# MaxMax2016/MixGAN-TTS

Hardware: AMD Instinct MI355X
Metric: denoiser steps/sec (80-mel, L=1000 frames, B=16 per GPU) (higher is better)
Workload: dtype f32

## Files before the change

### mixgan-tts_amd/csrc/denoiser_persist.h

```cpp
#pragma once
#include "common.h"
#include "denoiser_common.h"
#include "resblock_fused.h"

#define DP_SPIN_LIMIT (1u << 21)
#define DP_F_ROLES 1
#define DP_F_WITHHOLD 2

typedef unsigned long long dp_u64;
typedef __attribute__((address_space(1))) dp_u64 dp_gu64;
typedef __attribute__((address_space(1))) unsigned dp_gu32;
typedef __attribute__((address_space(1))) const char dp_gcchar;
typedef __attribute__((address_space(1))) const f32x4 dp_gcf32x4;

struct PersistArgs {
    const float *x_t;
    const float *cond;
    const float *cproj;
    float *cproj_out;
    const float *in_w, *in_b;
    const float *layers;
    size_t layer_stride, l_wc, l_w3, l_wo, l_bc, l_b3, l_bo;
    const float *p16layers;
    size_t p16layer_stride, p_wc, p_w3, p_wo;
    const float *skip_w, *skip_b, *out_w, *out_b;
    const float *hvec, *dvec;
    int vec_rows;
    float *out;
    const int64_t *t;
    const float *coef1, *coef2, *logvar;
    const float *noise;
    unsigned long long seed;
    unsigned long long noise_stream;
    float *x0_out;
    dp_u64 *gran;
    dp_u64 *team;
    unsigned *sync;
    unsigned *host_err;
    unsigned spin_limit;
    float *x0_save, *y_save, *skip_save;
    float *h_save, *g_save, *sig_save, *tnh_save;
    size_t act_stride;
    unsigned long long *dbg;
    int dbg_wave;
    int B, L, M, NL, tiles_per_b, post, clip, n_steps;
    int flags;
    float rsNL;
    int b_split;
    const float *x_t2, *hvec2, *dvec2, *cond2;
    float *out2;
};

struct DpIterK1 {
    static constexpr int N = 8, KW = 1;
    static __device__ __forceinline__ int chunk(int it) { return it; }
    static __device__ __forceinline__ int tap(int) { return 0; }
};
struct DpIterHead {
    static constexpr int N = 3, KW = 1;
    static __device__ __forceinline__ int chunk(int it) { return it; }
    static __device__ __forceinline__ int tap(int) { return 0; }
};
struct DpIterCentre {
    static constexpr int N = 8, KW = 3;
    static __device__ __forceinline__ int chunk(int it) { return it; }
    static __device__ __forceinline__ int tap(int) { return 1; }
};
struct DpIterOuter {
    static constexpr int N = 16, KW = 3;
    static __device__ __forceinline__ int chunk(int it) { return it >> 1; }
    static __device__ __forceinline__ int tap(int it) { return (it & 1) * 2; }
};

__device__ __forceinline__ int dp_pos(int ch) { return ((ch & 1) << 2) | ((ch >> 1) & 3); }
template <int NTC>
__device__ __forceinline__ int dp_at(int ch, int col) { return (((ch >> 3) * NTC + col) << 3) + dp_pos(ch); }

#ifndef DP_DIST_BIG
#define DP_DIST_BIG 3
#endif
template <int NMB, int NNB, int NTC, class IT, int DIST, bool SBASE>
__device__ __forceinline__ void dp_mfma_loop_at(f32x16 (&acc)[NMB][NNB], const f32x4 *const (&ap)[NMB], unsigned loff,
                                                const float *__restrict__ tile)
{
    static_assert(DIST >= 1 && DIST <= 3, "ring of 4 slots");
    f32x4 ring[4][NMB];
    f32x4 bb[2][NNB];
    dp_gcchar *ub[NMB];
    if (SBASE) {
#pragma unroll
        for (int i = 0; i < NMB; ++i) {
            const unsigned long long v = reinterpret_cast<unsigned long long>(ap[i]);
            const unsigned lo = __builtin_amdgcn_readfirstlane((unsigned)v), hi = __builtin_amdgcn_readfirstlane((unsigned)(v >> 32));
            ub[i] = (dp_gcchar *)(((unsigned long long)hi << 32) | lo);
        }
    }
    auto sbase = [&](int i, int qb) {
        dp_gcchar *p = ub[i] + (size_t)qb * 1024;
        asm volatile("" : "+s"(p));
        return p;
    };
    if (SBASE) asm volatile("" : "+v"(loff));
    auto wload = [&](int i, int qb, int d) -> f32x4 {
        if (SBASE) return *(dp_gcf32x4 *)(ub[i] + (size_t)qb * 1024 + loff + d * 1024);
        return ap[i][(size_t)(qb + d) * 64];
    };
    auto qbase = [](int it) { return (IT::chunk(it) * IT::KW + IT::tap(it)) * 4; };
    auto boff = [](int it) { return IT::chunk(it) * (4 * NTC * 8) + IT::tap(it) * 8; };
    {
        const int q0 = qbase(0);
#pragma unroll
        for (int s = 0; s < DIST; ++s)
#pragma unroll
            for (int i = 0; i < NMB; ++i) ring[s][i] = wload(i, q0, s);
        const float *T0 = tile + boff(0);
#pragma unroll
        for (int j = 0; j < NNB; ++j) bb[0][j] = *reinterpret_cast<const f32x4 *>(T0 + 32 * 8 * j);
    }
#pragma unroll 1
    for (int it = 0; it < IT::N; ++it) {
        const int itn = it + 1 < IT::N ? it + 1 : IT::N - 1;
        const int qc = qbase(it), qn = qbase(itn);
        const float *Tc = tile + boff(it), *Tn = tile + boff(itn);
        dp_gcchar *bc[NMB], *bn[NMB];
        if (SBASE) {
            asm volatile("" : "+v"(loff));
#pragma unroll
            for (int i = 0; i < NMB; ++i) {
                bc[i] = sbase(i, qc);
                bn[i] = sbase(i, qn);
            }
        }
#pragma unroll
        for (int u = 0; u < 4; ++u) {
#pragma unroll
            for (int i = 0; i < NMB; ++i) {
                constexpr int LIM = 4 - DIST;
                const int d = u < LIM ? u + DIST : u - LIM;
                if (SBASE) ring[(u + DIST) & 3][i] = *(dp_gcf32x4 *)((u < LIM ? bc[i] : bn[i]) + loff + d * 1024);
                else ring[(u + DIST) & 3][i] = wload(i, u < LIM ? qc : qn, d);
            }
            {
                const float *Tx = u < 3 ? Tc + (u + 1) * (NTC * 8) : Tn;
#pragma unroll
                for (int j = 0; j < NNB; ++j) bb[(u + 1) & 1][j] = *reinterpret_cast<const f32x4 *>(Tx + 32 * 8 * j);
            }
            __builtin_amdgcn_sched_barrier(0);
#pragma unroll
            for (int e = 0; e < 4; ++e) {
#pragma unroll
                for (int i = 0; i < NMB; ++i)
#pragma unroll
                    for (int j = 0; j < NNB; ++j)
                        acc[i][j] = __builtin_amdgcn_mfma_f32_32x32x2f32(ring[u][i][e], bb[u & 1][j][e], acc[i][j], 0, 0, 0);
                if (NMB * NNB < 4) __builtin_amdgcn_sched_barrier(0);
            }
            __builtin_amdgcn_sched_barrier(0);
        }
    }
}
template <int NMB, int NNB, int NTC, class IT, int DIST = (NMB * NNB >= 4 ? DP_DIST_BIG : 3)>
__device__ __forceinline__ void dp_mfma_loop(f32x16 (&acc)[NMB][NNB], const f32x4 *const (&ap)[NMB], const float *__restrict__ tile)
{
    dp_mfma_loop_at<NMB, NNB, NTC, IT, DIST, false>(acc, ap, 0u, tile);
}
template <int NMB, int NNB, int NTC, class IT, int DIST = (NMB * NNB >= 4 ? DP_DIST_BIG : 3)>
__device__ __forceinline__ void dp_mfma_loop_sbase(f32x16 (&acc)[NMB][NNB], const f32x4 *const (&ap)[NMB], unsigned loff,
                                             const float *__restrict__ tile)
{
    dp_mfma_loop_at<NMB, NNB, NTC, IT, DIST, true>(acc, ap, loff, tile);
}

template <int NTC, class F>
__device__ __forceinline__ void dp_store_block(float *T, int ch0, int col, int hh, F val)
{
#pragma unroll
    for (int q = 0; q < 4; ++q) {
        float *base = T + ((((ch0 >> 3) + q) * NTC + col) << 3);
        const f32x2 lo = {val(4 * q + 0), val(4 * q + 2)}, hi = {val(4 * q + 1), val(4 * q + 3)};
        *reinterpret_cast<f32x2 *>(base + 2 * hh) = lo;
        *reinterpret_cast<f32x2 *>(base + 4 + 2 * hh) = hi;
    }
}

__device__ __forceinline__ void dp_philox(unsigned long long seed, unsigned long long offset, unsigned long long idx,
                                          unsigned (&r)[4])
{
    unsigned c0 = (unsigned)idx, c1 = (unsigned)(idx >> 32), c2 = (unsigned)offset, c3 = (unsigned)(offset >> 32);
    unsigned k0 = (unsigned)seed, k1 = (unsigned)(seed >> 32);
#pragma unroll
    for (int i = 0; i < 10; ++i) {
        const unsigned long long p0 = (unsigned long long)0xD2511F53u * c0, p1 = (unsigned long long)0xCD9E8D57u * c2;
        const unsigned n0 = (unsigned)(p1 >> 32) ^ c1 ^ k0, n1 = (unsigned)p1, n2 = (unsigned)(p0 >> 32) ^ c3 ^ k1,
                       n3 = (unsigned)p0;
        c0 = n0; c1 = n1; c2 = n2; c3 = n3;
        k0 += 0x9E3779B9u;
        k1 += 0xBB67AE85u;
    }
    r[0] = c0; r[1] = c1; r[2] = c2; r[3] = c3;
}

__device__ __forceinline__ float dp_normal(unsigned long long seed, unsigned long long offset, unsigned long long idx)
{
    unsigned r[4];
    dp_philox(seed, offset, idx, r);
    const float u1 = ((float)r[0] + 1.0f) * 2.3283064365386963e-10f;
    const float u2 = (float)r[1] * 2.3283064365386963e-10f;
    return sqrtf(-2.0f * __logf(u1)) * __cosf(6.283185307179586f * u2);
}

#define DP_RLX_AGENT __ATOMIC_RELAXED, __HIP_MEMORY_SCOPE_AGENT

__device__ __forceinline__ void dp_fail(unsigned *sync, unsigned *host_err, unsigned code)
{
    __hip_atomic_store(sync + DP_SYNC_ERROR, code, DP_RLX_AGENT);
    if (host_err) __hip_atomic_store(host_err, code, __ATOMIC_RELAXED, __HIP_MEMORY_SCOPE_SYSTEM);
    __builtin_amdgcn_fence(__ATOMIC_RELEASE, "agent");
}
__device__ __forceinline__ bool dp_failed(unsigned *sync)
{
    __builtin_amdgcn_fence(__ATOMIC_ACQUIRE, "agent");
    return __hip_atomic_load(sync + DP_SYNC_ERROR, DP_RLX_AGENT) != 0u;
}
__device__ __forceinline__ void dp_take_ticket(int tid, unsigned *sync, unsigned &s_ticket, unsigned &s_launch, unsigned &s_dead)
{
    if (tid == 0) {
        s_ticket = __hip_atomic_fetch_add(sync + DP_SYNC_TICKET, 1u, DP_RLX_AGENT);
        s_launch = __hip_atomic_load(sync + DP_SYNC_LAUNCHES, DP_RLX_AGENT);
        s_dead = 0u;
    }
}
template <bool QUEUE_B>
__device__ __forceinline__ void dp_retire(int tid, unsigned *sync, int n_slots)
{
    if (tid == 0) {
        const unsigned done = __hip_atomic_fetch_add(sync + DP_SYNC_DONE, 1u, DP_RLX_AGENT);
        if (done == (unsigned)n_slots - 1u) {
            __hip_atomic_store(sync + DP_SYNC_DONE, 0u, DP_RLX_AGENT);
            __hip_atomic_store(sync + DP_SYNC_TICKET, 0u, DP_RLX_AGENT);
            if (QUEUE_B) __hip_atomic_store(sync + DP_SYNC_TICKET_B, 0u, DP_RLX_AGENT);
            __hip_atomic_fetch_add(sync + DP_SYNC_LAUNCHES, 1u, DP_RLX_AGENT);
        }
    }
}
#define DP_EPOCH(launch_no, NL, step) ((launch_no) * ((unsigned)(NL) + 1u) + (unsigned)(step) + 1u)

struct DpPosterior { float c1, c2, sg; };
__device__ __forceinline__ DpPosterior dp_posterior_at(const PersistArgs &a, int b)
{
    long tb = (long)a.t[b];
    tb = tb < 0 ? 0 : (tb >= a.n_steps ? a.n_steps - 1 : tb);
    const float c1 = a.coef1[tb], c2 = a.coef2[tb];
    const float sg = tb == 0 ? 0.f : __expf(0.5f * a.logvar[tb]);
    return {c1, c2, sg};
}
__device__ __forceinline__ float dp_clip_x0(float x0, int clip)
{
    if (clip) x0 = fminf(fmaxf(x0, -1.f), 1.f);
    return x0;
}
__device__ __forceinline__ float dp_posterior(const DpPosterior &p, float x0, float xt, float nz) { return fmaf(p.sg, nz, fmaf(p.c1, x0, p.c2 * xt)); }
#define DP_STAMP(k) do { if (TIMING && tid == 64 * a.dbg_wave) a.dbg[((size_t)tile * (a.NL + 2) + stamp_row) * 12 + (k)] = clock64(); } while (0)

template <int NT, int RW>
__device__ __forceinline__ void dp_cproj_fetch(const float *cp, float *cl, int w, int lane, int l0, int L)
{
    constexpr int LPR = NT / 4;
    constexpr int RPI = 64 / LPR;
    const int rsub = lane / LPR, c4 = lane - rsub * LPR;
    unsigned off = (unsigned)(((RW * w + rsub) * L + min(l0 + 4 * c4, L - 4)) * 4);
    asm volatile("" : "+v"(off));
    float *dst = cl + (size_t)RW * w * NT;
    const unsigned at = (unsigned)(size_t)(__attribute__((address_space(3))) void *)dst;
#pragma unroll
    for (int it = 0; it < RW / RPI; ++it) {
        const float *gi = cp + (size_t)it * RPI * L;
        const unsigned m = __builtin_amdgcn_readfirstlane(at + (unsigned)(it * RPI * NT * 4));
        asm volatile("s_mov_b32 m0, %0\n\ts_nop 0\n\tglobal_load_lds_dwordx4 %1, %2" : : "s"(m), "v"(off), "s"(gi) : "memory");
    }
}

template <int NT, bool VEC4, bool TIMING = false, bool SAVE = false, int NWV = NT / 8, int CPM = 0, bool SOLO = false>
__global__ __launch_bounds__(NWV * 64, ((NT == 64 && NWV == 4) || SOLO) ? 1 : 2) void denoiser_persist_kernel(PersistArgs a)
{
    static_assert(!SOLO || (NT == 32 && NWV == 4), "SOLO is the one-per-CU build of the 4-wave 32-frame form");
    static_assert(!(CPM && SAVE), "the saving forward computes its projections and keeps none");
    constexpr bool READP = CPM == 2, WRITEP = CPM == 1;
#ifndef DP_DIST_SOLO
#define DP_DIST_SOLO 2
#endif
    constexpr int DBIG = ((NT == 64 && NWV == 4) || SOLO) ? DP_DIST_SOLO : DP_DIST_BIG;
#ifndef DP_ONEPASS_WHEN
#define DP_ONEPASS_WHEN (MB == 2 && ((NT == 64 && NWV == 4) || SOLO))
#endif
    static_assert((NT == 32 && (NWV == 4 || NWV == 8)) || (NT == 64 && (NWV == 8 || NWV == 4)),
                  "tile widths: 32 frames (4 waves, two workgroups per CU; or 8 waves, one per CU) or 64 (8 waves, one)");
    constexpr int NTHR = NWV * 64, NW = NWV;
    constexpr bool TWO_PER_CU = NT == 32 && NWV == 4;
    constexpr int MB = 8 / NW;
    constexpr bool ONEPASS = DP_ONEPASS_WHEN;
    constexpr int NNB = NT / 32;
    constexpr int NC = NT, NH = NT + 2;
    __shared__ __attribute__((aligned(16))) float lds[RB_C * (NC + NH)];
    __shared__ unsigned s_tile, s_dead, s_launch;
    float *condT = lds;
    float *hT = lds + RB_C * NC;

    const int tid = threadIdx.x, lane = tid & 63, w = tid >> 6;
    const int hh = lane >> 5, c32 = lane & 31;
    const int L = a.L;
    const int wu = __builtin_amdgcn_readfirstlane(w);
    const unsigned loff = (unsigned)lane * 16u;

    const int n_tiles = a.tiles_per_b * a.B;
    const unsigned hw_id = __builtin_amdgcn_s_getreg((31 << 11) | 4);
    const int role = (TWO_PER_CU && (a.flags & DP_F_ROLES)) ? (int)(hw_id & 1u) : 0;
    if (tid == 0) {
        const int nA = (TWO_PER_CU && (a.flags & DP_F_ROLES)) ? (a.B / 2) * a.tiles_per_b : n_tiles;
        const int n_mine = role == 0 ? nA : n_tiles - nA;
        unsigned tk = __hip_atomic_fetch_add(a.sync + (role ? DP_SYNC_TICKET_B : DP_SYNC_TICKET), 1u, DP_RLX_AGENT);
        int tl;
        if ((int)tk < n_mine) tl = (role == 0 ? 0 : nA) + (int)tk;
        else {
            tk = __hip_atomic_fetch_add(a.sync + (role ? DP_SYNC_TICKET : DP_SYNC_TICKET_B), 1u, DP_RLX_AGENT);
            tl = (role == 0 ? nA : 0) + (int)tk;
        }
        s_tile = (unsigned)tl;
        s_launch = __hip_atomic_load(a.sync + DP_SYNC_LAUNCHES, DP_RLX_AGENT);
        s_dead = 0u;
    }
    __syncthreads();
    const int tile = min((int)s_tile, n_tiles - 1);
    const unsigned launch_no = s_launch;
    const int bg = tile / a.tiles_per_b, jt = tile - bg * a.tiles_per_b;
    const bool second = a.b_split > 0 && bg >= a.b_split;
    const int b = second ? bg - a.b_split : bg;
    const int Bp = a.b_split > 0 ? (second ? a.B - a.b_split : a.b_split) : a.B;
    const bool do_save = SAVE && (a.b_split == 0 || second);
    const float *const x_in = second ? a.x_t2 : a.x_t;
    float *const x_out = second ? a.out2 : a.out;
    const int l0 = jt * NT;
    const bool has_left = jt > 0, has_right = jt + 1 < a.tiles_per_b;
    int stamp_row = 0;
    DP_STAMP(0);
    if (TIMING && tid == 0) {
        a.dbg[((size_t)tile * (a.NL + 2)) * 12 + 2] = hw_id;
        a.dbg[((size_t)tile * (a.NL + 2)) * 12 + 3] = __builtin_amdgcn_s_getreg((31 << 11) | 20);
    }

    {
        const float *cb = (second ? a.cond2 : a.cond) + (size_t)b * RB_C * L;
        if (READP) {
            if (VEC4) dp_cproj_fetch<NT, 32 * MB>(a.cproj + (size_t)b * a.NL * RB_C * L, lds, w, lane, l0, L);
        } else if (VEC4) {
#pragma unroll
            for (int k = 0; k < 64 * NT / NTHR; ++k) {
                const int idx = tid + k * NTHR;
                const int row = idx / (NT / 4), c4 = idx - row * (NT / 4);
                const int f0 = l0 + 4 * c4;
                const bool ok = f0 < L;
                const f32x4 v = *reinterpret_cast<const f32x4 *>(cb + (size_t)row * L + min(f0, L - 4));
#pragma unroll
                for (int e = 0; e < 4; ++e) condT[dp_at<NC>(row, 4 * c4 + e)] = ok ? v[e] : 0.f;
            }
        } else {
#pragma unroll
            for (int k = 0; k < 256 * NT / NTHR; ++k) {
                const int idx = tid + k * NTHR;
                const int row = idx / NT, cc = idx - row * NT;
                const int f = l0 + cc;
                const float v = cb[(size_t)row * L + min(f, L - 1)];
                condT[dp_at<NC>(row, cc)] = f < L ? v : 0.f;
            }
        }
        const float *xb = x_in + (size_t)b * a.M * L;
#pragma unroll
        for (int k = 0; k < 96 * NT / NTHR; ++k) {
            const int idx = tid + k * NTHR;
            const int row = idx / NT, c = idx - row * NT;
            const int f = l0 + c;
            const float v = xb[(size_t)min(row, a.M - 1) * L + min(f, L - 1)];
            hT[dp_at<NH>(row, c)] = (row < a.M && f < L) ? v : 0.f;
        }
    }

    f32x16 st[2 * MB][NNB];
    const int rbase = 32 * MB * w;
    auto row_of = [&](int i, int r) { return rbase + 32 * i + 8 * (r >> 2) + 4 * hh + (r & 3); };
#pragma unroll
    for (int i = 0; i < MB; ++i)
#pragma unroll
        for (int j = 0; j < NNB; ++j)
#pragma unroll
            for (int r = 0; r < 16; ++r) {
                st[i][j][r] = a.in_b[row_of(i, r)];
                st[MB + i][j][r] = 0.f;
            }
    __syncthreads();
    {
        f32x16 acc[MB][NNB];
        const f32x4 *ap[MB];
#pragma unroll
        for (int i = 0; i < MB; ++i) {
            ap[i] = reinterpret_cast<const f32x4 *>(a.in_w) + (size_t)(MB * wu + i) * 12 * 64;
#pragma unroll
            for (int j = 0; j < NNB; ++j) acc[i][j] = st[i][j];
        }
        dp_mfma_loop_sbase<MB, NNB, NH, DpIterHead>(acc, ap, loff, hT + c32 * 8 + hh * 4);
#pragma unroll
        for (int i = 0; i < MB; ++i)
#pragma unroll
            for (int j = 0; j < NNB; ++j)
#pragma unroll
                for (int r = 0; r < 16; ++r) st[i][j][r] = fmaxf(acc[i][j][r], 0.f);
    }
    DP_STAMP(1);
    bool fvalid[NNB];
    const size_t bbase = (size_t)b * RB_C * L;
    auto save_block = [&](float *dst, int ch0, int j, auto val) {
        const int f = l0 + 32 * j + c32;
        if (f < L) {
#pragma unroll
            for (int r = 0; r < 16; ++r) dst[bbase + (size_t)(ch0 + 8 * (r >> 2) + 4 * hh + (r & 3)) * L + f] = val(r);
        }
    };
#pragma unroll
    for (int j = 0; j < NNB; ++j) fvalid[j] = l0 + 32 * j + c32 < L;
    if (SAVE && do_save) {
#pragma unroll
        for (int i = 0; i < MB; ++i)
#pragma unroll
            for (int j = 0; j < NNB; ++j) save_block(a.x0_save, rbase + 32 * i, j, [&](int r) { return st[i][j][r]; });
    }
    dp_gu64 *const gran = (dp_gu64 *)a.gran;

    for (int l = 0; l < a.NL; ++l) {
        const float *lp = a.layers + (size_t)l * a.layer_stride;
        const size_t vrows = a.vec_rows ? (size_t)a.vec_rows : (size_t)Bp;
        const float *hv = (second ? a.hvec2 : a.hvec) + ((size_t)l * vrows + b) * RB_C;
        const float *dv = (second ? a.dvec2 : a.dvec) + ((size_t)l * vrows + b) * RB_C;
        const unsigned epoch = DP_EPOCH(launch_no, a.NL, l);
        const int par = l & 1;
        stamp_row = l + 1;
        DP_STAMP(0);

        f32x16 acc1[MB][NNB];
        if (READP && VEC4) {
            asm volatile("s_waitcnt vmcnt(0)" ::: "memory");
#pragma unroll
            for (int i = 0; i < MB; ++i)
#pragma unroll
                for (int j = 0; j < NNB; ++j)
#pragma unroll
                    for (int r = 0; r < 16; ++r) acc1[i][j][r] = lds[row_of(i, r) * NT + 32 * j + c32];
        } else if (READP) {
            const float *cp = a.cproj + ((size_t)b * a.NL + l) * RB_C * L;
#pragma unroll
            for (int i = 0; i < MB; ++i)
#pragma unroll
                for (int j = 0; j < NNB; ++j) {
                    unsigned lo = (unsigned)((rbase + 4 * hh) * L + min(l0 + 32 * j + c32, L - 1));
                    asm volatile("" : "+v"(lo));
#pragma unroll
                    for (int r = 0; r < 16; ++r) acc1[i][j][r] = cp[lo + (unsigned)((32 * i + 8 * (r >> 2) + (r & 3)) * L)];
                }
        } else {
#pragma unroll
            for (int i = 0; i < MB; ++i)
#pragma unroll
                for (int j = 0; j < NNB; ++j)
#pragma unroll
                    for (int r = 0; r < 16; ++r) acc1[i][j][r] = lp[a.l_bc + row_of(i, r)];
            const f32x4 *wc = reinterpret_cast<const f32x4 *>(lp + a.l_wc);
            const f32x4 *ap[MB];
#pragma unroll
            for (int i = 0; i < MB; ++i) ap[i] = wc + (size_t)(MB * wu + i) * 32 * 64;
            dp_mfma_loop_sbase<MB, NNB, NC, DpIterK1, (MB * NNB >= 4 ? DBIG : 3)>(acc1, ap, loff, condT + c32 * 8 + hh * 4);
            if (WRITEP) {
                float *co = a.cproj_out + ((size_t)b * a.NL + l) * RB_C * L;
                unsigned lo = (unsigned)((rbase + 4 * hh) * L + l0 + c32);
                asm volatile("" : "+v"(lo));
#pragma unroll
                for (int i = 0; i < MB; ++i)
#pragma unroll
                    for (int j = 0; j < NNB; ++j)
                        if (l0 + 32 * j + c32 < L) {
#pragma unroll
                            for (int r = 0; r < 16; ++r)
                                co[lo + (unsigned)((32 * i + 8 * (r >> 2) + (r & 3)) * L + 32 * j)] = acc1[i][j][r];
                        }
            }
        }
#pragma unroll
        for (int i = 0; i < MB; ++i)
#pragma unroll
            for (int j = 0; j < NNB; ++j)
#pragma unroll
                for (int r = 0; r < 16; ++r) acc1[i][j][r] += st[i][j][r] + hv[row_of(i, r)];
        DP_STAMP(1);
        f32x16 acc2[MB][2][NNB];
#pragma unroll
        for (int p = 0; p < MB; ++p)
#pragma unroll
            for (int r = 0; r < 16; ++r) {
                const int ch = row_of(p, r);
                const float bg = lp[a.l_b3 + ch], bf = lp[a.l_b3 + RB_C + ch];
#pragma unroll
                for (int j = 0; j < NNB; ++j) {
                    acc2[p][0][j][r] = bg;
                    acc2[p][1][j][r] = bf;
                }
            }
        __syncthreads();
        DP_STAMP(2);
#pragma unroll
        for (int i = 0; i < MB; ++i)
#pragma unroll
            for (int j = 0; j < NNB; ++j)
            {
                dp_store_block<NH>(hT, rbase + 32 * i, 1 + 32 * j + c32, hh,
                                   [&](int r) { return fvalid[j] ? acc1[i][j][r] : 0.f; });
                if (SAVE && do_save) save_block(a.h_save + (size_t)l * a.act_stride, rbase + 32 * i, j, [&](int r) { return acc1[i][j][r]; });
            }
        if (READP && VEC4 && l + 1 < a.NL)
            dp_cproj_fetch<NT, 32 * MB>(a.cproj + ((size_t)b * a.NL + l + 1) * RB_C * L, lds, w, lane, l0, L);
        __syncthreads();
        DP_STAMP(3);

        if (w < 2) {
            bool go = w == 0 ? has_left : has_right;
            if ((a.flags & DP_F_WITHHOLD) && w == 0 && jt == 1) go = false;
            if (go) {
                const int dst_tile = w == 0 ? tile - 1 : tile + 1;
                const int col = w == 0 ? 1 : NT;
                dp_gu64 *g = gran + (((size_t)par * n_tiles + dst_tile) * 2 + (w == 0 ? 1 : 0)) * RB_C;
#pragma unroll
                for (int k = 0; k < 4; ++k) {
                    const int row = lane + 64 * k;
                    const dp_u64 v = ((dp_u64)epoch << 32) | (dp_u64)__float_as_uint(hT[dp_at<NH>(row, col)]);
                    __hip_atomic_store(g + row, v, DP_RLX_AGENT);
                }
            }
        }

        const f32x4 *w3 = reinterpret_cast<const f32x4 *>(lp + a.l_w3);
        const f32x4 *ap2[MB][2];
#pragma unroll
        for (int p = 0; p < MB; ++p) {
            ap2[p][0] = w3 + (size_t)(2 * (MB * wu + p)) * 96 * 64;
            ap2[p][1] = w3 + (size_t)(2 * (MB * wu + p) + 1) * 96 * 64;
        }
        if (ONEPASS) {
            dp_mfma_loop_sbase<2 * MB, NNB, NH, DpIterCentre, DBIG>(reinterpret_cast<f32x16 (&)[2 * MB][NNB]>(acc2),
                                                              reinterpret_cast<const f32x4 *const (&)[2 * MB]>(ap2), loff,
                                                              hT + c32 * 8 + hh * 4);
        } else {
#pragma unroll
            for (int p = 0; p < MB; ++p)
                dp_mfma_loop_sbase<2, NNB, NH, DpIterCentre, (2 * NNB >= 4 ? DBIG : 3)>(acc2[p], ap2[p], loff, hT + c32 * 8 + hh * 4);
        }
        DP_STAMP(4);

        if (w < 2) {
            const bool from = w == 0 ? has_left : has_right;
            const int col = w == 0 ? 0 : NT + 1;
            unsigned v[4] = {0u, 0u, 0u, 0u};
            if (from && s_dead == 0u) {
                dp_gu64 *g = gran + (((size_t)par * n_tiles + tile) * 2 + w) * RB_C;
                unsigned spins = 0;
                for (;;) {
                    bool ok = true;
#pragma unroll
                    for (int k = 0; k < 4; ++k) {
                        const dp_u64 x = __hip_atomic_load(g + lane + 64 * k, DP_RLX_AGENT);
                        v[k] = (unsigned)x;
                        ok &= (unsigned)(x >> 32) == epoch;
                    }
                    if (__all(ok)) break;
                    if (++spins > a.spin_limit) {
                        if (lane == 0) {
                            dp_fail(a.sync, a.host_err, 1u + (unsigned)l);
                            s_dead = 1u;
                        }
                        break;
                    }
                    __builtin_amdgcn_s_sleep(8);
                }
            }
#pragma unroll
            for (int k = 0; k < 4; ++k) hT[dp_at<NH>(lane + 64 * k, col)] = from ? __uint_as_float(v[k]) : 0.f;
        }
        DP_STAMP(5);
        __syncthreads();
        DP_STAMP(6);

        if (ONEPASS) {
            dp_mfma_loop_sbase<2 * MB, NNB, NH, DpIterOuter, DBIG>(reinterpret_cast<f32x16 (&)[2 * MB][NNB]>(acc2),
                                                             reinterpret_cast<const f32x4 *const (&)[2 * MB]>(ap2), loff,
                                                             hT + c32 * 8 + hh * 4);
        } else {
#pragma unroll
            for (int p = 0; p < MB; ++p)
                dp_mfma_loop_sbase<2, NNB, NH, DpIterOuter, (2 * NNB >= 4 ? DBIG : 3)>(acc2[p], ap2[p], loff, hT + c32 * 8 + hh * 4);
        }
        DP_STAMP(7);
        __syncthreads();
        DP_STAMP(8);
#pragma unroll
        for (int p = 0; p < MB; ++p)
#pragma unroll
            for (int j = 0; j < NNB; ++j)
            {
                if (SAVE && do_save) {
#pragma unroll
                    for (int r = 0; r < 16; ++r) {
                        acc2[p][0][j][r] = mg_sigmoid(acc2[p][0][j][r]);
                        acc2[p][1][j][r] = mg_tanh(acc2[p][1][j][r]);
                    }
                    const size_t lo = (size_t)l * a.act_stride;
                    save_block(a.sig_save + lo, rbase + 32 * p, j, [&](int r) { return acc2[p][0][j][r]; });
                    save_block(a.tnh_save + lo, rbase + 32 * p, j, [&](int r) { return acc2[p][1][j][r]; });
                    save_block(a.g_save + lo, rbase + 32 * p, j, [&](int r) { return acc2[p][0][j][r] * acc2[p][1][j][r]; });
                    dp_store_block<NH>(hT, rbase + 32 * p, 32 * j + c32, hh, [&](int r) { return acc2[p][0][j][r] * acc2[p][1][j][r]; });
                } else {
                    dp_store_block<NH>(hT, rbase + 32 * p, 32 * j + c32, hh,
                                       [&](int r) { return mg_sigmoid(acc2[p][0][j][r]) * mg_tanh(acc2[p][1][j][r]); });
                }
            }
#pragma unroll
        for (int i = 0; i < MB; ++i)
#pragma unroll
            for (int j = 0; j < NNB; ++j)
#pragma unroll
                for (int r = 0; r < 16; ++r) {
                    const int row = row_of(i, r);
                    st[i][j][r] += lp[a.l_bo + row] + dv[row];
                    st[MB + i][j][r] += lp[a.l_bo + RB_C + row];
                }
        DP_STAMP(9);
        __syncthreads();
        DP_STAMP(10);

        {
            const f32x4 *wo = reinterpret_cast<const f32x4 *>(lp + a.l_wo);
            const f32x4 *ap[2 * MB];
#pragma unroll
            for (int i = 0; i < MB; ++i) {
                ap[i] = wo + (size_t)(MB * wu + i) * 32 * 64;
                ap[MB + i] = wo + (size_t)(8 + MB * wu + i) * 32 * 64;
            }
            dp_mfma_loop_sbase<2 * MB, NNB, NH, DpIterK1, (2 * MB * NNB >= 4 ? DBIG : 3)>(st, ap, loff, hT + c32 * 8 + hh * 4);
        }
        DP_STAMP(11);
#pragma unroll
        for (int i = 0; i < MB; ++i)
#pragma unroll
            for (int j = 0; j < NNB; ++j)
#pragma unroll
                for (int r = 0; r < 16; ++r) st[i][j][r] *= 0.70710678118654752440f;
    }

    stamp_row = a.NL + 1;
    DP_STAMP(0);
    __syncthreads();
#pragma unroll
    for (int i = 0; i < MB; ++i)
#pragma unroll
        for (int j = 0; j < NNB; ++j)
            {
                dp_store_block<NH>(hT, rbase + 32 * i, 32 * j + c32, hh, [&](int r) { return st[MB + i][j][r] * a.rsNL; });
                if (SAVE && do_save) save_block(a.skip_save, rbase + 32 * i, j, [&](int r) { return st[MB + i][j][r]; });
            }
    __syncthreads();
    {
        f32x16 acc[MB][NNB];
        const f32x4 *ap[MB];
#pragma unroll
        for (int i = 0; i < MB; ++i) {
            ap[i] = reinterpret_cast<const f32x4 *>(a.skip_w) + (size_t)(MB * wu + i) * 32 * 64;
#pragma unroll
            for (int j = 0; j < NNB; ++j)
#pragma unroll
                for (int r = 0; r < 16; ++r) acc[i][j][r] = a.skip_b[row_of(i, r)];
        }
        dp_mfma_loop_sbase<MB, NNB, NH, DpIterK1>(acc, ap, loff, hT + c32 * 8 + hh * 4);
#pragma unroll
        for (int i = 0; i < MB; ++i)
#pragma unroll
            for (int j = 0; j < NNB; ++j)
            {
                dp_store_block<NC>(condT, rbase + 32 * i, 32 * j + c32, hh, [&](int r) { return fmaxf(acc[i][j][r], 0.f); });
                if (SAVE && do_save) save_block(a.y_save, rbase + 32 * i, j, [&](int r) { return fmaxf(acc[i][j][r], 0.f); });
            }
    }
    __syncthreads();
    const int mblocks = (a.M + 31) / 32;
    for (int task = wu; task < mblocks * NNB; task += NW) {
        const int mb = task / NNB, nb = task - mb * NNB;
        f32x16 o[1][1];
#pragma unroll
        for (int r = 0; r < 16; ++r) {
            const int row = 32 * mb + 8 * (r >> 2) + 4 * hh + (r & 3);
            o[0][0][r] = row < a.M ? a.out_b[row] : 0.f;
        }
        const f32x4 *const ap[1] = {reinterpret_cast<const f32x4 *>(a.out_w) + (size_t)mb * 32 * 64};
        dp_mfma_loop_sbase<1, 1, NC, DpIterK1>(o, ap, loff, condT + (32 * nb + c32) * 8 + hh * 4);
        const int f = l0 + 32 * nb + c32;
        const size_t bo = (size_t)b * a.M * L;
        const bool bad = dp_failed(a.sync);
        const float poison = __builtin_nanf("");
        if (!a.post) {
#pragma unroll
            for (int r = 0; r < 16; ++r) {
                const int row = 32 * mb + 8 * (r >> 2) + 4 * hh + (r & 3);
                if (row < a.M && f < L) x_out[bo + (size_t)row * L + f] = bad ? poison : o[0][0][r];
            }
        } else {
            const DpPosterior ps = dp_posterior_at(a, b);
            const unsigned long long seed = a.seed, off = (a.noise_stream << 32) | (unsigned long long)launch_no;
            const int fc = min(f, L - 1);
            float xt[16], nz[16];
#pragma unroll
            for (int r = 0; r < 16; ++r) {
                const int row = min(32 * mb + 8 * (r >> 2) + 4 * hh + (r & 3), a.M - 1);
                const size_t e = bo + (size_t)row * L + fc;
                xt[r] = a.x_t[e];
                nz[r] = a.noise ? a.noise[e] : dp_normal(seed, off, e);
            }
#pragma unroll
            for (int r = 0; r < 16; ++r) {
                const int row = 32 * mb + 8 * (r >> 2) + 4 * hh + (r & 3);
                if (row < a.M && f < L) {
                    const size_t e = bo + (size_t)row * L + f;
                    float x0 = o[0][0][r];
                    if (a.x0_out) a.x0_out[e] = x0;
                    x0 = dp_clip_x0(x0, a.clip);
                    a.out[e] = bad ? poison : dp_posterior(ps, x0, xt[r], nz[r]);
                }
            }
        }
    }
    DP_STAMP(1);
    dp_retire<true>(tid, a.sync, n_tiles);
}
```

Before: 382.2.

## Peel tail iteration, carry scalar bases, and interleave loads with MFMAs in sbase loop

Restructures the scalar-base MFMA inner loop. The last iteration is peeled so it skips the redundant prefetch loads. Next-chunk weight base pointers are carried across iterations as scalar adds instead of being recomputed each time. Sched_group_barrier hints spread global and LDS loads between MFMAs instead of issuing them all before a hard barrier. This aims to cut wasted loads, scalar address math and issue stalls, but it adds template complexity and the scheduling hints may change register pressure.

```diff
diff --git a/mixgan-tts_amd/csrc/denoiser_persist.h b/mixgan-tts_amd/csrc/denoiser_persist.h
--- a/mixgan-tts_amd/csrc/denoiser_persist.h
+++ b/mixgan-tts_amd/csrc/denoiser_persist.h
@@ -79,6 +79,30 @@
 #ifndef DP_DIST_BIG
 #define DP_DIST_BIG 3
 #endif
+#ifndef DP_KL_SKIP_TAIL
+#define DP_KL_SKIP_TAIL 1
+#endif
+#ifndef DP_KL_CARRY
+#define DP_KL_CARRY 2
+#endif
+#ifndef DP_KL_SPREAD
+#define DP_KL_SPREAD 1
+#endif
+template <int NG, int NL, int NM>
+__device__ __forceinline__ void dp_spread_group()
+{
+#if DP_KL_SPREAD
+#pragma unroll
+    for (int m = 0; m < NG + NL; ++m) {
+        __builtin_amdgcn_sched_group_barrier(0x008, DP_KL_SPREAD, 0);
+        if (m < NG) __builtin_amdgcn_sched_group_barrier(0x020, 1, 0);
+        else __builtin_amdgcn_sched_group_barrier(0x100, 1, 0);
+    }
+    __builtin_amdgcn_sched_group_barrier(0x008, NM - DP_KL_SPREAD * (NG + NL), 0);
+#endif
+}
+struct dp_false { static constexpr bool value = false; };
+struct dp_true { static constexpr bool value = true; };
 template <int NMB, int NNB, int NTC, class IT, int DIST, bool SBASE>
 __device__ __forceinline__ void dp_mfma_loop_at(f32x16 (&acc)[NMB][NNB], const f32x4 *const (&ap)[NMB], unsigned loff,
                                                 const float *__restrict__ tile)
@@ -117,35 +141,88 @@
 #pragma unroll
         for (int j = 0; j < NNB; ++j) bb[0][j] = *reinterpret_cast<const f32x4 *>(T0 + 32 * 8 * j);
     }
+    if constexpr (!SBASE) {
 #pragma unroll 1
-    for (int it = 0; it < IT::N; ++it) {
-        const int itn = it + 1 < IT::N ? it + 1 : IT::N - 1;
+        for (int it = 0; it < IT::N; ++it) {
+            const int itn = it + 1 < IT::N ? it + 1 : IT::N - 1;
+            const int qc = qbase(it), qn = qbase(itn);
+            const float *Tc = tile + boff(it), *Tn = tile + boff(itn);
+#pragma unroll
+            for (int u = 0; u < 4; ++u) {
+#pragma unroll
+                for (int i = 0; i < NMB; ++i) {
+                    constexpr int LIM = 4 - DIST;
+                    const int d = u < LIM ? u + DIST : u - LIM;
+                    ring[(u + DIST) & 3][i] = wload(i, u < LIM ? qc : qn, d);
+                }
+                {
+                    const float *Tx = u < 3 ? Tc + (u + 1) * (NTC * 8) : Tn;
+#pragma unroll
+                    for (int j = 0; j < NNB; ++j) bb[(u + 1) & 1][j] = *reinterpret_cast<const f32x4 *>(Tx + 32 * 8 * j);
+                }
+                __builtin_amdgcn_sched_barrier(0);
+#pragma unroll
+                for (int e = 0; e < 4; ++e) {
+#pragma unroll
+                    for (int i = 0; i < NMB; ++i)
+#pragma unroll
+                        for (int j = 0; j < NNB; ++j)
+                            acc[i][j] = __builtin_amdgcn_mfma_f32_32x32x2f32(ring[u][i][e], bb[u & 1][j][e], acc[i][j], 0, 0, 0);
+                    if (NMB * NNB < 4) __builtin_amdgcn_sched_barrier(0);
+                }
+                __builtin_amdgcn_sched_barrier(0);
+            }
+        }
+        return;
+    }
+    constexpr bool SKIP_TAIL = DP_KL_SKIP_TAIL != 0, CARRY = DP_KL_CARRY != 0;
+    constexpr bool SPREAD = DP_KL_SPREAD != 0 && NMB * NNB >= 4;
+    dp_gcchar *bcur[NMB];
+    if (CARRY) {
+#pragma unroll
+        for (int i = 0; i < NMB; ++i) bcur[i] = sbase(i, qbase(0));
+    }
+    auto body = [&](const int it, auto tail) {
+        constexpr bool TAIL = decltype(tail)::value;
+        constexpr int LIM = 4 - DIST;
+        const int itn = (SKIP_TAIL || it + 1 < IT::N) ? it + 1 : IT::N - 1;
         const int qc = qbase(it), qn = qbase(itn);
         const float *Tc = tile + boff(it), *Tn = tile + boff(itn);
         dp_gcchar *bc[NMB], *bn[NMB];
-        if (SBASE) {
-            asm volatile("" : "+v"(loff));
+        auto next_bases = [&]() {
+            const long long dq = (long long)(qn - qc) * 1024;
 #pragma unroll
             for (int i = 0; i < NMB; ++i) {
+                bn[i] = bc[i] + dq;
+                asm volatile("" : "+s"(bn[i]));
+            }
+        };
+        asm volatile("" : "+v"(loff));
+#pragma unroll
+        for (int i = 0; i < NMB; ++i) {
+            if (CARRY) bc[i] = bcur[i];
+            else {
                 bc[i] = sbase(i, qc);
-                bn[i] = sbase(i, qn);
-            }
-        }
+                if (!TAIL) bn[i] = sbase(i, qn);
+            }
+        }
+        if (CARRY && !TAIL && DP_KL_CARRY == 1) next_bases();
 #pragma unroll
         for (int u = 0; u < 4; ++u) {
-#pragma unroll
-            for (int i = 0; i < NMB; ++i) {
-                constexpr int LIM = 4 - DIST;
-                const int d = u < LIM ? u + DIST : u - LIM;
-                if (SBASE) ring[(u + DIST) & 3][i] = *(dp_gcf32x4 *)((u < LIM ? bc[i] : bn[i]) + loff + d * 1024);
-                else ring[(u + DIST) & 3][i] = wload(i, u < LIM ? qc : qn, d);
-            }
-            {
+            if (!(TAIL && u >= LIM)) {
+#pragma unroll
+                for (int i = 0; i < NMB; ++i) {
+                    const int d = u < LIM ? u + DIST : u - LIM;
+                    ring[(u + DIST) & 3][i] = *(dp_gcf32x4 *)((u < LIM ? bc[i] : bn[i]) + loff + d * 1024);
+                }
+            }
+            if (!(TAIL && u == 3)) {
                 const float *Tx = u < 3 ? Tc + (u + 1) * (NTC * 8) : Tn;
 #pragma unroll
                 for (int j = 0; j < NNB; ++j) bb[(u + 1) & 1][j] = *reinterpret_cast<const f32x4 *>(Tx + 32 * 8 * j);
             }
-            __builtin_amdgcn_sched_barrier(0);
+            if (!SPREAD) __builtin_amdgcn_sched_barrier(0);
+            if (CARRY && !TAIL && DP_KL_CARRY == 2 && u == 0) next_bases();
 #pragma unroll
             for (int e = 0; e < 4; ++e) {
 #pragma unroll
@@ -155,8 +232,26 @@
                         acc[i][j] = __builtin_amdgcn_mfma_f32_32x32x2f32(ring[u][i][e], bb[u & 1][j][e], acc[i][j], 0, 0, 0);
                 if (NMB * NNB < 4) __builtin_amdgcn_sched_barrier(0);
             }
+            if (SPREAD) {
+                const bool g = !(TAIL && u >= LIM), l = !(TAIL && u == 3);
+                if (g && l) dp_spread_group<NMB, NNB, 4 * NMB * NNB>();
+                else if (g) dp_spread_group<NMB, 0, 4 * NMB * NNB>();
+                else if (l) dp_spread_group<0, NNB, 4 * NMB * NNB>();
+            }
             __builtin_amdgcn_sched_barrier(0);
         }
+        if (CARRY && !TAIL) {
+#pragma unroll
+            for (int i = 0; i < NMB; ++i) bcur[i] = bn[i];
+        }
+    };
+    if (SKIP_TAIL) {
+#pragma unroll 1
+        for (int it = 0; it < IT::N - 1; ++it) body(it, dp_false{});
+        body(IT::N - 1, dp_true{});
+    } else {
+#pragma unroll 1
+        for (int it = 0; it < IT::N; ++it) body(it, dp_false{});
     }
 }
 template <int NMB, int NNB, int NTC, class IT, int DIST = (NMB * NNB >= 4 ? DP_DIST_BIG : 3)>
```

Result: no change. 385.8, median of 6 (+0.9%).
